# qinzheng93/GeoTransformer

Hardware: NVIDIA H100
Metric: point-cloud pairs/sec (3DMatch-shape synth) (higher is better)
Workload: dtype f32

## Files before the change

geotransformer_b200/_lib.py:

```python
import ctypes
import os
import threading

import torch

_HERE = os.path.dirname(os.path.abspath(__file__))
LIB_PATH = os.path.join(_HERE, 'libgeob200.so')
_lib = None

c_void_p, c_int64, c_int32, c_float, c_double, c_size_t, c_int = (
    ctypes.c_void_p, ctypes.c_int64, ctypes.c_int32, ctypes.c_float, ctypes.c_double, ctypes.c_size_t, ctypes.c_int)

SIGNATURES = {}


def _sig(name, restype, *argtypes):
    SIGNATURES[name] = (restype, list(argtypes))


P, I64, I32, F, D, SZ = c_void_p, c_int64, c_int32, c_float, c_double, c_size_t
_sig('geob200_last_error', ctypes.c_char_p)
_sig('geob200_launch_count', ctypes.c_uint64)
_sig('geob200_grid_subsample_workspace_bytes', SZ, I64, I64)
_sig('geob200_grid_subsample', c_int, P, I64, P, I64, F, P, P, P, SZ, P)
# ... 91 lines not shown
_sig('geob200_feature_corr_indices', c_int, P, P, P, P, I64, I64, I32, P, P, P, P, P)
_sig('geob200_ransac_features_batched_workspace_bytes', SZ, I64, I64, I64, I64, I64)
_sig('geob200_ransac_features_batched', c_int, P, P, P, P, I64, I64, I64, I64, P, P, F, I64, I64, I64, ctypes.c_uint64, I64, P, P, P, P, P,
     P, P, P, P, P, P, P, P, P, SZ, P)
_sig('geob200_correspondence_metrics_batched_workspace_bytes', SZ, I64, I64)
_sig('geob200_correspondence_metrics_batched', c_int, P, P, I64, I64, P, P, I64, F, P, I64, P, SZ, P)
_sig('geob200_corr_order_batched', c_int, P, I64, I64, P, I64, P, P)
_sig('geob200_corr_select_batched', c_int, P, P, P, I64, I64, P, P, I64, I64, P, P, P, P, P)
_sig('geob200_sparse_correspondence_eval_batched_workspace_bytes', SZ, I64, I64, I64)
_sig('geob200_sparse_correspondence_eval_batched', c_int, P, P, I64, P, P, I64, P, I64, I64, I64, P, P, SZ, P)
_sig('geob200_registration_error_batched', c_int, P, I64, P, I64, P, P, I64, c_int, D, D, P, P)
_sig('geob200_weighted_procrustes_counts', c_int, P, P, P, I64, I64, P, F, F, P, P)

_sig('geob200_linear_profile_enable', c_int, c_int)
_sig('geob200_set_split_k', c_int, c_int)
_sig('geob200_set_linear_persistent', c_int, c_int)
_sig('geob200_linear_profile_read', I64, I64, P, P)
_sig('geob200_backbone_workspace_bytes', SZ, P, P)
_sig('geob200_backbone_forward_batched', c_int, P, P, P, P, P, P, P, P, P, P, P, P, SZ, P, SZ, P, I64, P, P)
_sig('geob200_cloud_max_count', c_int, P, I64, I64, I64, I64, P, P, P)
_sig('geob200_transformer_batched_workspace_bytes', SZ, I64, P, I64, I64, I64)
_sig('geob200_transformer_forward_batched', c_int, P, I64, I64, I64, P, I64, P, P, P, P, SZ, P)
_sig('geob200_attention_batched_workspace_bytes', SZ, P, I64, I64)
_sig('geob200_attention_batched', c_int, P, I64, I64, I64, I64, I64, I64, I64, P, SZ, P)
_sig('geob200_attention_batched_keeps_probs', c_int, P, I64, I64, I64)
_sig('geob200_superpoint_targets_batched_workspace_bytes', SZ, I64)
_sig('geob200_superpoint_targets_batched', c_int, P, P, P, I64, P, F, I64, ctypes.c_uint64, ctypes.c_uint64, I64, P, P, P, P, SZ, P)
_sig('geob200_nonfinite_check', c_int, P, P, I64, I64, P, P)
_sig('geob200_batch_loss_weights', c_int, P, I64, I64, P, P, P, P, P)
_sig('geob200_kpconv_group_norm_batched', c_int, P, P, P, P, I64, I64, I64, P, I64, P, P, I64, I64, F, I64, P, P, F, c_int, F, P, P, P,
# ... 82 lines not shown
```

geotransformer_b200/csrc/common.cuh:

```cuda
#pragma once
#include <cuda_runtime.h>
#include <stdint.h>
#include <stdio.h>

namespace geob200 {

void set_error(const char* fmt, ...);
void count_launches(int n);
int ensure_max_smem(const void* kernel);

#define GEOB_CHECK_CUDA(expr)                                                                   \
    do {                                                                                        \
        cudaError_t _e = (expr);                                                                \
        if (_e != cudaSuccess) {                                                                \
            geob200::set_error("%s:%d CUDA error %s: %s", __FILE__, __LINE__, #expr,            \
                               cudaGetErrorString(_e));                                         \
            return -1;                                                                          \
        }                                                                                       \
    } while (0)

#define GEOB_CHECK_LAUNCH()                                                                     \
    do {                                                                                        \
        cudaError_t _e = cudaGetLastError();                                                    \
        if (_e != cudaSuccess) {                                                                \
// ... 39 lines not shown
    return v[0];
}

struct GnFuse {
    int groups;
    int slot_width;
    double* partial;
};

constexpr int GEOB_MAX_CLOUDS = 64;
struct GnSeg {
    int n_clouds;
    int n_pairs;
    int start[GEOB_MAX_CLOUDS + 1];
};
size_t fused_group_norm_workspace_bytes_batched(int64_t n_rows, int64_t channels, int64_t groups, int64_t n_pairs);
int group_norm_impl(const float* x, int64_t n_rows, int64_t channels, int64_t groups, const float* gamma, const float* beta, float eps,
                    const float* residual, int leaky, float slope, float* y, void* workspace, size_t workspace_bytes, void* stream,
                    const GnSeg* seg);
int linear_group_norm_impl(const float* x, int64_t ldx, const float* weight, const float* bias, int64_t m, int64_t n, int64_t k,
                           int64_t groups, const float* gamma, const float* beta, float eps, const float* residual, int leaky,
                           float slope, float* pre_norm, float* y, void* workspace, size_t workspace_bytes, void* stream,
                           const GnSeg* seg, const float* w_img = nullptr);
int kpconv_group_norm_impl(const float* s_feats, const float* q_points, const float* s_points, const int64_t* neighbors,
                           int64_t n_query, int64_t n_support, int64_t n_neighbors, const float* kernel_points, int64_t n_kernel,
                           const float* weights_t, const float* bias, int64_t c_in, int64_t c_out, float sigma, int64_t groups,
                           const float* gamma, const float* beta, float eps, int leaky, float slope, float* pre_norm, float* y,
                           void* gn_workspace, size_t gn_workspace_bytes, void* workspace, size_t workspace_bytes, void* stream,
                           const GnSeg* seg, const float* w_img = nullptr);
int linear_img(const float* x, int64_t ldx, const float* weight, const float* w_img, const float* bias, float* y, int64_t ldy,
               int64_t m, int64_t n, int64_t k, int relu, void* stream);
int kpconv_tc_impl(const float* s_feats, const float* q_points, const float* s_points, const int64_t* neighbors, int64_t n_query,
                   int64_t n_support, int64_t n_neighbors, const float* kernel_points, int64_t n_kernel, const float* weights_t,
                   const float* w_img, const float* bias, int64_t c_in, int64_t c_out, float sigma, float* out, void* workspace,
                   size_t workspace_bytes, void* stream);

int maxpool_seg(const float* x, const int64_t* neighbors, int64_t n_query, int64_t n_support, int64_t n_neighbors, int64_t channels,
                float* y, const GnSeg* seg, const int* cloud_max, void* stream);

struct Segs {
    int n;
    int max;
    int start[GEOB_MAX_CLOUDS];
    int count[GEOB_MAX_CLOUDS];
};
int segs_from_counts(Segs* s, int64_t n, const int64_t* counts);
// ... 54 lines not shown
```

geotransformer_b200/csrc/kpconv.cu:

```cuda
#include "common.cuh"
#include "geob200.h"
#include "kpconv.cuh"

namespace geob200 {

constexpr int TQ = 32;
constexpr int CC = 32;

__global__ void __launch_bounds__(256) kpconv_c1_kernel(const float* __restrict__ feats, const float* __restrict__ q_pts,
                                                        const float* __restrict__ s_pts, const long long* __restrict__ nbr,
                                                        int H, const float* __restrict__ kp, const float* __restrict__ W,
                                                        const float* __restrict__ bias, float sigma, int Ns, int M, int Cout,
                                                        float* __restrict__ out) {
    __shared__ float kp_s[KP * 3];
    __shared__ float wk_s[16][KP_PAD];
    __shared__ float np_s[16];
    if (threadIdx.x < KP * 3) kp_s[threadIdx.x] = kp[threadIdx.x];
    __syncthreads();
    const int lane = threadIdx.x & 31, warp = threadIdx.x >> 5;
    const int sub = lane >> 4, sl = lane & 15;
    const int slot = warp * 2 + sub;
    const int m = blockIdx.x * 16 + slot;
    const bool live = m < M;
    float acc[KP];
// ... 781 lines not shown
    const int lane = threadIdx.x & 31;
    const int m = blockIdx.x * 8 + (threadIdx.x >> 5);
    if (m >= M) return;
    const long long idx = up[(long long)m * up_stride];
    float* yr = y + (long long)m * (C1 + C2);
    for (int c = lane; c < C1; c += 32) yr[c] = (idx < Ns) ? x[idx * C1 + c] : 0.f;
    if (skip != nullptr)
        for (int c = lane; c < C2; c += 32) yr[C1 + c] = skip[(long long)m * C2 + c];
}

}

using namespace geob200;

namespace geob200 {
int linear_tc(const float* x, int64_t ldx, const float* w, int64_t ldw, const float* w_img, const float* bias, const float* row_scale, float* y, int64_t ldy,
              int64_t m, int64_t n, int64_t k, int relu, cudaStream_t st, const GnFuse* gn = nullptr);
static int g_linear_mode = 1;
}

extern "C" {

void geob200_set_linear_mode(int mode) { g_linear_mode = mode; }

size_t geob200_kpconv_workspace_bytes(int64_t n_support) { return (size_t)n_support + 256; }

size_t geob200_kpconv_tc_workspace_bytes(int64_t n_query, int64_t n_support, int64_t c_in) {
    return align_up((size_t)n_support, 256) + align_up((size_t)n_query * 4, 256) + (size_t)n_query * KP * (size_t)c_in * 4 + 1024;
}

int geob200_kpconv_tc(const float* s_feats, const float* q_points, const float* s_points, const int64_t* neighbors, int64_t n_query,
                      int64_t n_support, int64_t n_neighbors, const float* kernel_points, int64_t n_kernel, const float* weights_t,
// ... 18 lines not shown
    Arena ar(workspace, workspace_bytes);
    unsigned char* pos = ar.take<unsigned char>(n_support);
    float* inv_count = ar.take<float>(n_query);
    float* wf = ar.take<float>((size_t)n_query * KP * c_in);
    row_positive_kernel<<<(unsigned)((n_support + 7) / 8), 256, 0, st>>>(s_feats, (int)n_support, (int)c_in, pos);
    launch_kpconv_gather(s_feats, pos, q_points, s_points, (const long long*)neighbors, (int)n_neighbors, kernel_points, sigma,
                         (int)n_support, (int)n_query, (int)c_in, wf, inv_count, st);
    GEOB_CHECK_LAUNCH();
    count_launches(2);
    const int rc = linear_tc(wf, KP * c_in, weights_t, KP * c_in, w_img, bias, inv_count, out, c_out, n_query, c_out, KP * c_in, 0, st);
    GEOB_REQUIRE(rc == 0, "kpconv_tc: tensor-core GEMM rejected the shape");
    return 0;
}

int linear_img(const float* x, int64_t ldx, const float* weight, const float* w_img, const float* bias, float* y, int64_t ldy,
               int64_t m, int64_t n, int64_t k, int relu, void* stream) {
    if (g_linear_mode == 1 && m > 0 && n > 0 && k > 0) {
        const int rc = linear_tc(x, ldx, weight, k, w_img, bias, nullptr, y, ldy, m, n, k, relu, (cudaStream_t)stream);
        if (rc <= 0) return rc;
    }
    return geob200_linear(x, ldx, weight, bias, y, ldy, m, n, k, relu, stream);
}
}

extern "C" {

int geob200_kpconv(const float* s_feats, const float* q_points, const float* s_points, const int64_t* neighbors,
                   int64_t n_query, int64_t n_support, int64_t n_neighbors, const float* kernel_points, int64_t n_kernel,
                   const float* weights, const float* bias, int64_t c_in, int64_t c_out, float sigma, float* out,
                   void* workspace, size_t workspace_bytes, void* stream) {
    cudaStream_t st = (cudaStream_t)stream;
// ... 193 lines not shown
    return 0;
}

int geob200_linear_group_norm(const float* x, int64_t ldx, const float* weight, const float* bias, int64_t m, int64_t n, int64_t k,
                              int64_t groups, const float* gamma, const float* beta, float eps, const float* residual, int leaky,
                              float slope, float* pre_norm, float* y, void* workspace, size_t workspace_bytes, void* stream) {
    return geob200::linear_group_norm_impl(x, ldx, weight, bias, m, n, k, groups, gamma, beta, eps, residual, leaky, slope, pre_norm, y,
                                           workspace, workspace_bytes, stream, nullptr);
}
}

namespace geob200 {
int linear_group_norm_impl(const float* x, int64_t ldx, const float* weight, const float* bias, int64_t m, int64_t n, int64_t k,
                           int64_t groups, const float* gamma, const float* beta, float eps, const float* residual, int leaky,
                           float slope, float* pre_norm, float* y, void* workspace, size_t workspace_bytes, void* stream,
                           const GnSeg* seg, const float* w_img) {
    cudaStream_t st = (cudaStream_t)stream;
    const int64_t np = (seg != nullptr && seg->n_pairs > 1) ? seg->n_pairs : 1;
    GEOB_REQUIRE(m > 0 && n > 0 && k > 0 && groups > 0 && n % groups == 0 && n % 4 == 0, "linear_group_norm: bad shape");
    GEOB_REQUIRE(workspace_bytes >= (np > 1 ? fused_group_norm_workspace_bytes_batched(m, n, groups, np)
                                            : geob200_fused_group_norm_workspace_bytes(m, n, groups)), "linear_group_norm: workspace too small");
    if (g_linear_mode == 1) {
        const GnWs w = gn_carve(workspace, workspace_bytes, groups, np);
        GnFuse gn{(int)groups, 0, w.partial};
        const int rc = linear_tc(x, ldx, weight, k, w_img, bias, nullptr, pre_norm, n, m, n, k, 0, st, &gn);
        if (rc < 0) return rc;
        if (rc == 0) {
            if (np > 1) {
                launch_gn_seg_apply(pre_norm, w, gamma, beta, residual, y, m, n, groups, eps, leaky, slope, *seg, st);
            } else {
                launch_gn_apply(pre_norm, w, gamma, beta, residual, y, m, n, groups, eps, leaky, slope, st);
                count_launches(2);
            }
            GEOB_CHECK_LAUNCH();
            return 0;
        }
    }
    int rc = linear_img(x, ldx, weight, w_img, bias, pre_norm, n, m, n, k, 0, stream);
    if (rc != 0) return rc;
    return group_norm_impl(pre_norm, m, n, groups, gamma, beta, eps, residual, leaky, slope, y, workspace, workspace_bytes, stream, seg);
}
// ... 152 lines not shown
```

geotransformer_b200/csrc/linear_tc.cu:

```cuda
#include <cuda.h>

#include <cstdlib>
#include <mutex>
#include <vector>

#include "common.cuh"
#include "geob200.h"
#include "hopper.cuh"

namespace geob200 {
namespace ltc {

using namespace hop;

constexpr int BM = 128;
constexpr int KC = 32;
constexpr int TILE_A = BM * 128;
constexpr int TILE_B = 128 * 128;
constexpr int STAGE = TILE_A + 2 * TILE_B;
constexpr int NSTAGE = 4;
constexpr int PRODUCER_WARP = 8;
constexpr int NTHREADS = (PRODUCER_WARP + 4) * 32;
constexpr int SMEM = NSTAGE * STAGE + 1024 + 256 + 8 * 128 * 8 + 512;

__global__ void __launch_bounds__(256) split_tf32_kernel(const float* __restrict__ w, long long ld, long long n, long long k,
                                                         float* __restrict__ out) {
    const long long nk = n * k;
    for (long long i = (long long)blockIdx.x * blockDim.x + threadIdx.x; i < nk; i += (long long)gridDim.x * blockDim.x) {
        const long long r = i / k, c = i % k;
        const float x = w[r * ld + c];
        const float hi = tf32_rn(x);
        out[i] = hi;
        out[nk + i] = x - hi;
    }
}

template <int BNI>
__global__ void __launch_bounds__(NTHREADS, 1) linear_tc_kernel(const __grid_constant__ CUtensorMap map_x,
                                                                const __grid_constant__ CUtensorMap map_w,
                                                                const float* __restrict__ bias, const float* __restrict__ row_scale,
                                                                float* __restrict__ Y, int ldy, int M, int N, int K, int BN, int relu,
                                                                GnFuse gn, float* __restrict__ splitk_out, int chunks_per_split,
                                                                int col_tiles, int row_tiles, int num_tiles) {
    constexpr int R = BNI / 2;
    extern __shared__ unsigned char smem_raw[];
    unsigned char* smem = (unsigned char*)(((uintptr_t)smem_raw + 1023) & ~(uintptr_t)1023);
    uint64_t* bars = (uint64_t*)(smem + NSTAGE * STAGE);
    uint64_t* full = bars;
    uint64_t* empty = bars + NSTAGE;
    float2* gn_sm = (float2*)(smem + NSTAGE * STAGE + 256);
    float* bias_s = (float*)(gn_sm + 8 * 128);
    const int warp = threadIdx.x >> 5, lane = threadIdx.x & 31;
    const int nk = (K + KC - 1) / KC;
    const int tiles_per_split = col_tiles * row_tiles;

    if (threadIdx.x == 0) {
        for (int s = 0; s < NSTAGE; ++s) { mbar_init(&full[s], 1); mbar_init(&empty[s], 8); }
        asm volatile("fence.mbarrier_init.release.cluster;" ::: "memory");
// ... 29 lines not shown
    const int wg = warp >> 2, wq = warp & 3;
    int s = 0;
    uint32_t ph = 0;
    for (int t = blockIdx.x; t < num_tiles; t += gridDim.x) {
        const int z = t / tiles_per_split, rem = t % tiles_per_split;
        const int ty = rem / col_tiles;
        const int m0 = ty * BM, n0 = (rem % col_tiles) * BN;
        const int kc0 = z * chunks_per_split, kc1 = min(nk, kc0 + chunks_per_split);
        asm volatile("bar.sync 1, 256;" ::: "memory");
        if (threadIdx.x < 128) bias_s[threadIdx.x] = (bias != nullptr && (int)threadIdx.x < BN) ? __ldg(bias + n0 + threadIdx.x) : 0.f;
        asm volatile("bar.sync 1, 256;" ::: "memory");

        float acc[R], cor[R];
#pragma unroll
        for (int i = 0; i < R; ++i) { acc[i] = 0.f; cor[i] = 0.f; }
        const int g = lane >> 2, tq = lane & 3;
        const int a_off = (wg * 64 + wq * 16 + g) * 128 + tq * 4;
        for (int kc = kc0; kc < kc1; ++kc) {
            mbar_wait(&full[s], ph);
            unsigned char* st = smem + s * STAGE;
            uint32_t f[2][KC / 8][4];
#pragma unroll
            for (int kk = 0; kk < KC / 8; ++kk)
#pragma unroll
                for (int e = 0; e < 4; ++e) {
                    const int j = 2 * kk + (e >> 1);
                    const float x = *reinterpret_cast<const float*>(st + a_off + (e & 1) * 8 * 128 + ((j ^ g) << 4));
                    const float hi = tf32_rn(x);
                    f[0][kk][e] = __float_as_uint(hi);
                    f[1][kk][e] = __float_as_uint(x - hi);
                }
            const uint32_t sb = smem_u32(st + TILE_A);
            const uint64_t b_hi = make_desc(sb), b_lo = make_desc(sb + TILE_B);
            wgmma_fence();
#pragma unroll
            for (int kk = 0; kk < KC / 8; ++kk) {
                const uint64_t adv = (uint64_t)(kk * 2);
                const uint32_t accum = (kc == kc0 && kk == 0) ? 0u : 1u;
                wgmma_tf32_rs<BNI>(acc, f[0][kk], b_hi + adv, accum);
                wgmma_tf32_rs<BNI>(cor, f[0][kk], b_lo + adv, accum);
                wgmma_tf32_rs<BNI>(cor, f[1][kk], b_hi + adv, 1u);
            }
            wgmma_commit();
            wgmma_wait<0>();
            __syncwarp();
            if (lane == 0) mbar_arrive(&empty[s]);
            if (++s == NSTAGE) { s = 0; ph ^= 1u; }
        }
        reg_fence(acc);
        reg_fence(cor);

        const int r0 = m0 + wg * 64 + wq * 16 + (lane >> 2);
        const int c0 = 2 * (lane & 3);
        float rs[2];
#pragma unroll
        for (int h = 0; h < 2; ++h) rs[h] = (row_scale != nullptr && r0 + 8 * h < M) ? row_scale[r0 + 8 * h] : 1.0f;
        if (splitk_out != nullptr) {
#pragma unroll
            for (int j = 0; j < BNI / 8; ++j)
#pragma unroll
                for (int h = 0; h < 2; ++h) {
                    const int m = r0 + 8 * h, col = 8 * j + c0;
                    if (m < M && col < BN)
                        *reinterpret_cast<float2*>(splitk_out + ((long long)z * M + m) * N + n0 + col) =
                            make_float2(acc[4 * j + 2 * h] + cor[4 * j + 2 * h], acc[4 * j + 2 * h + 1] + cor[4 * j + 2 * h + 1]);
                }
            continue;
        }
// ... 105 lines not shown
    cuuint32_t box[2] = {(cuuint32_t)KC, (cuuint32_t)box_rows};
    cuuint32_t estr[2] = {1, 1};
    CUresult r = fn(map, CU_TENSOR_MAP_DATA_TYPE_FLOAT32, 2, (void*)base, gdim, gstride, box, estr, CU_TENSOR_MAP_INTERLEAVE_NONE,
                    CU_TENSOR_MAP_SWIZZLE_128B, CU_TENSOR_MAP_L2_PROMOTION_L2_128B, CU_TENSOR_MAP_FLOAT_OOB_FILL_NONE);
    if (r != CUDA_SUCCESS) { set_error("cuTensorMapEncodeTiled failed with CUresult %d", (int)r); return -1; }
    return 0;
}

}

struct ProfRec { cudaEvent_t a, b; long long m, n, k; };
static std::vector<ProfRec> g_prof;
static std::mutex g_prof_mu;
static bool g_prof_on = false;
static bool g_splitk_on = true;
static bool g_persistent_on = true;

struct StreamWs { void* ptr; size_t bytes; };
static std::vector<std::pair<cudaStream_t, StreamWs>> g_split_ws, g_wimg_ws;
static std::mutex g_split_mu;
static float* stream_scratch(std::vector<std::pair<cudaStream_t, StreamWs>>& pool, cudaStream_t st, size_t bytes) {
    std::lock_guard<std::mutex> lk(g_split_mu);
    for (auto& e : pool)
        if (e.first == st) {
            if (e.second.bytes >= bytes) return (float*)e.second.ptr;
            cudaFreeAsync(e.second.ptr, st);
            e.second = {nullptr, 0};
            if (cudaMallocAsync(&e.second.ptr, bytes * 2, st) != cudaSuccess) return nullptr;
            e.second.bytes = bytes * 2;
            return (float*)e.second.ptr;
// ... 2 lines not shown
    const size_t cap = bytes * 2 > (16u << 20) ? bytes * 2 : (16u << 20);
    if (cudaMallocAsync(&w.ptr, cap, st) != cudaSuccess) return nullptr;
    w.bytes = cap;
    pool.push_back({st, w});
    return (float*)w.ptr;
}

static void launch_split_tf32(const float* w, int64_t ld, int64_t n, int64_t k, float* out, cudaStream_t st) {
    const long long nk = (long long)n * k;
    long long blocks = (nk + 255) / 256;
    if (blocks > 4LL * num_sms()) blocks = 4LL * num_sms();
    ltc::split_tf32_kernel<<<(unsigned)(blocks > 0 ? blocks : 1), 256, 0, st>>>(w, ld, n, k, out);
    count_launches(1);
}

int linear_tc(const float* x, int64_t ldx, const float* w, int64_t ldw, const float* w_img, const float* bias, const float* row_scale,
              float* y, int64_t ldy, int64_t m, int64_t n, int64_t k, int relu, cudaStream_t st, const GnFuse* gn) {
    if (m < 64 || n < 32 || (n % 16) != 0 || (k % 4) != 0 || (ldx % 4) != 0) return 1;
    if ((reinterpret_cast<uintptr_t>(x) & 15) || (reinterpret_cast<uintptr_t>(w_img) & 15)) return 1;
    if (w_img == nullptr && ((ldw % 4) != 0 || (reinterpret_cast<uintptr_t>(w) & 15))) return 1;
    if (n > 128 && (n % 128) != 0) return 1;
    const int BN = (int)(n >= 128 ? 128 : n);
    const int col_tiles = (int)(n / BN), row_tiles = (int)((m + ltc::BM - 1) / ltc::BM);
    GnFuse g{};
    if (gn != nullptr) {
        g = *gn;
        const int64_t cpg = n / g.groups;
        if (g.groups <= 0 || n % g.groups != 0 || (cpg < 32 ? (32 % cpg) != 0 : (cpg % 32) != 0 || (BN % cpg) != 0) || relu) return 1;
        g.slot_width = (int)(cpg < 32 ? cpg : 32);
    }
    const int nk = (int)((k + ltc::KC - 1) / ltc::KC);
    const int tiles = col_tiles * row_tiles;
    int splits = 1;
    if (g_splitk_on && tiles * 2 <= num_sms() && nk >= 16) {
        splits = nk / 8;
        if (splits > num_sms() / tiles) splits = num_sms() / tiles;
        if (splits > 16) splits = 16;
        if (splits < 2) splits = 1;
    }
    if (gn != nullptr && splits > 1) return 1;
    int cps = nk;
    float* part = nullptr;
    if (splits > 1) {
        cps = (nk + splits - 1) / splits;
        splits = (nk + cps - 1) / cps;
        part = stream_scratch(g_split_ws, st, (size_t)splits * (size_t)m * (size_t)n * sizeof(float));
        if (part == nullptr) { splits = 1; cps = nk; }
    }
    float* img = nullptr;
    if (w_img == nullptr) {
        img = stream_scratch(g_wimg_ws, st, (size_t)2 * (size_t)n * (size_t)k * sizeof(float));
        if (img == nullptr) { set_error("linear_tc: weight image scratch allocation failed"); return -1; }
        w_img = img;
    }
    CUtensorMap mx, mw;
    if (ltc::encode_map(&mx, x, m, k, ldx, ltc::BM)) return -1;
    if (ltc::encode_map(&mw, w_img, 2 * n, k, k, BN)) return -1;
    ProfRec rec{};
    const bool prof = g_prof_on;
    if (prof) {
        cudaEventCreate(&rec.a);
        cudaEventCreate(&rec.b);
        rec.m = m; rec.n = n; rec.k = k;
        cudaEventRecord(rec.a, st);
    }
    if (img != nullptr) launch_split_tf32(w, ldw, n, k, img, st);
    const int num_tiles = tiles * splits;
    const bool persistent = g_persistent_on && splits == 1 && tiles > num_sms();
    const unsigned grid = (unsigned)(persistent ? num_sms() : num_tiles);
    const void* kern = BN <= 32 ? (const void*)ltc::linear_tc_kernel<32> : BN <= 64 ? (const void*)ltc::linear_tc_kernel<64>
                                                                                      : (const void*)ltc::linear_tc_kernel<128>;
    if (ensure_max_smem(kern)) return -1;
#define GEOB_LTC_LAUNCH(BNI)                                                                                                  \
    ltc::linear_tc_kernel<BNI><<<grid, ltc::NTHREADS, ltc::SMEM, st>>>(mx, mw, bias, row_scale, y, (int)ldy, (int)m, (int)n, (int)k, \
                                                                       BN, relu, g, part, cps, col_tiles, row_tiles, num_tiles)
    if (BN <= 32) GEOB_LTC_LAUNCH(32);
    else if (BN <= 64) GEOB_LTC_LAUNCH(64);
    else GEOB_LTC_LAUNCH(128);
#undef GEOB_LTC_LAUNCH
    if (part != nullptr) {
        const long long mn = (long long)m * n;
        ltc::splitk_reduce_kernel<<<(unsigned)((mn / 4 + 255) / 256), 256, 0, st>>>(part, splits, mn, (int)n, bias, row_scale, y, (int)ldy, relu);
        count_launches(1);
    }
    if (prof) {
        cudaEventRecord(rec.b, st);
        std::lock_guard<std::mutex> lk(g_prof_mu);
        g_prof.push_back(rec);
    }
    GEOB_CHECK_LAUNCH();
    count_launches(1);
    return 0;
}

}

extern "C" {

int geob200_set_linear_persistent(int on) {
    geob200::g_persistent_on = on != 0;
    return 0;
}

int geob200_split_tf32(const float* w, int64_t ld, int64_t n, int64_t k, float* out, void* stream) {
    GEOB_REQUIRE(n > 0 && k > 0 && ld >= k, "split_tf32: bad shape (%lld x %lld, ld %lld)", (long long)n, (long long)k, (long long)ld);
    geob200::launch_split_tf32(w, ld, n, k, out, (cudaStream_t)stream);
    GEOB_CHECK_LAUNCH();
    return 0;
}

int geob200_set_split_k(int on) {
    geob200::g_splitk_on = on != 0;
    return 0;
}

int geob200_linear_profile_enable(int on) {
    std::lock_guard<std::mutex> lk(geob200::g_prof_mu);
    for (auto& r : geob200::g_prof) { cudaEventDestroy(r.a); cudaEventDestroy(r.b); }
    geob200::g_prof.clear();
    geob200::g_prof_on = on != 0;
    return 0;
}

int64_t geob200_linear_profile_read(int64_t capacity, int64_t* shapes, float* ms) {
    std::lock_guard<std::mutex> lk(geob200::g_prof_mu);
    int64_t n = 0;
    for (auto& r : geob200::g_prof) {
        if (n >= capacity) break;
        if (cudaEventSynchronize(r.b) != cudaSuccess) break;
// ... 11 lines not shown
```

geotransformer_b200/csrc/native.cu:

```cuda
#include "common.cuh"
#include "geob200.h"

namespace geob200 {

struct Ctx {
    Arena ar;
    void* gn_ws;
    size_t gn_ws_bytes;
    void* stream;
    int groups;
    Ctx(void* p, size_t n) : ar(p, n) {}
    float* fl(int64_t rows, int64_t ch) { return ar.take<float>((size_t)rows * (size_t)ch); }
};

#define TRY(expr)                  \
    do {                           \
        int _rc = (expr);          \
        if (_rc != 0) return _rc;  \
    } while (0)

static int run_kpconv(Ctx& c, const geob200_kpconv_t& k, const float* s_feats, const float* q_pts, const float* s_pts,
                      const int64_t* nbr, int64_t m, int64_t ns, int64_t h, float* out) {
    const bool tc = (k.c_in % 32 == 0) && (k.c_out % 16 == 0) && k.c_out >= 32 && (k.c_out <= 128 || k.c_out % 128 == 0) && m >= 64 &&
                    k.weights_t != nullptr;
// ... 27 lines not shown
        const size_t wb = geob200_kpconv_tc_workspace_bytes(m, ns, k.c_in);
        const size_t mark = c.ar.off;
        void* ws = c.ar.take<char>(wb);
        GEOB_REQUIRE(c.ar.ok(), "native: arena too small (kpconv)");
        TRY(kpconv_group_norm_impl(s_feats, q_pts, s_pts, nbr, m, ns, h, k.kernel_points, 15, k.weights_t, k.bias, k.c_in, k.c_out,
                                   k.sigma, c.groups, n.gamma, n.beta, 1e-5f, 1, 0.1f, y, out, c.gn_ws, c.gn_ws_bytes, ws, wb, c.stream, seg,
                                   k.weights_img));
        c.ar.off = mark;
        return 0;
    }
    TRY(run_kpconv(c, k, s_feats, q_pts, s_pts, nbr, m, ns, h, y));
    return group_norm_impl(y, m, k.c_out, c.groups, n.gamma, n.beta, 1e-5f, nullptr, 1, 0.1f, out, c.gn_ws, c.gn_ws_bytes, c.stream, seg);
}

static int run_unary(Ctx& c, const geob200_linear_t& l, const geob200_norm_t& n, const float* x, int64_t rows, const float* residual,
                     int leaky, float* out, const GnSeg* seg) {
    float* t = c.fl(rows, l.c_out);
    GEOB_REQUIRE(c.ar.ok(), "native: arena too small (unary)");
    TRY(linear_group_norm_impl(x, l.c_in, l.weight, l.bias, rows, l.c_out, l.c_in, c.groups, n.gamma, n.beta, 1e-5f, residual, leaky,
                               0.1f, t, out, c.gn_ws, c.gn_ws_bytes, c.stream, seg, l.weight_img));
    return 0;
}

static int run_resblock(Ctx& c, const geob200_resblock_t& b, const float* feats, int64_t ns, const float* q_pts, const float* s_pts,
                        const int64_t* nbr, int64_t m, int64_t h, float* out, const GnSeg* seg_s, const GnSeg* seg_q,
                        const int* cloud_max = nullptr) {
    const float* x = feats;
    if (b.has_unary1) {
        float* u = c.fl(ns, b.unary1.c_out);
        TRY(run_unary(c, b.unary1, b.norm1, feats, ns, nullptr, 1, u, seg_s));
        x = u;
    }
    float* yn = c.fl(m, b.conv.c_out);
    GEOB_REQUIRE(c.ar.ok(), "native: arena too small (resblock)");
    TRY(run_kpconv_norm(c, b.conv, b.norm_conv, x, q_pts, s_pts, nbr, m, ns, h, yn, seg_q));
    const float* sc = feats;
// ... 78 lines not shown
                         sg[lvl - 1], sg[lvl], sub_cloud_max != nullptr ? sub_cloud_max[lvl - 1] : nullptr));
        const geob200_resblock_t& b2 = net->blocks[bi++];
        float* o2 = c.fl(m, b2.unary2.c_out);
        TRY(run_resblock(c, b2, o1, m, points[lvl], points[lvl], neighbors[lvl], m, neighbor_width[lvl], o2, sg[lvl], sg[lvl]));
        const geob200_resblock_t& b3 = net->blocks[bi++];
        float* o3 = (lvl == S - 1) ? out_feats[0] : c.fl(m, b3.unary2.c_out);
        TRY(run_resblock(c, b3, o2, m, points[lvl], points[lvl], neighbors[lvl], m, neighbor_width[lvl], o3, sg[lvl], sg[lvl]));
        enc[lvl] = o3; enc_ch[lvl] = b3.unary2.c_out;
    }
    const float* latent = enc[S - 1];
    int64_t latent_ch = enc_ch[S - 1];
    int oi = 1;
    for (int lvl = S - 1; lvl >= net->finest_decoder; --lvl) {
        const int64_t m = level_rows[lvl - 1], ns = level_rows[lvl];
        const int64_t c2 = enc_ch[lvl - 1];
        float* cat = c.fl(m, latent_ch + c2);
        GEOB_REQUIRE(c.ar.ok(), "native: arena too small (decoder)");
        TRY(geob200_upsample_concat(latent, upsampling[lvl - 1], upsampling_width[lvl - 1], ns, enc[lvl - 1], m, latent_ch, c2, cat, stream));
        const geob200_linear_t& l = net->decoders[S - 1 - lvl];
        float* o = out_feats[oi++];
        if (lvl == net->finest_decoder) {
            TRY(linear_img(cat, l.c_in, l.weight, l.weight_img, l.bias, o, l.c_out, m, l.c_out, l.c_in, 0, stream));
        } else {
            TRY(run_unary(c, l, net->decoder_norms[S - 1 - lvl], cat, m, nullptr, 1, o, sg[lvl - 1]));
        }
        latent = o; latent_ch = l.c_out;
    }
    GEOB_REQUIRE(c.ar.ok(), "native: arena too small");
    return 0;
}


static int run_tail(Ctx& c, const geob200_tlayer_t& L, const float* hidden, const float* inp, int64_t rows, int64_t ch, float* out) {
    float* h = c.fl(rows, ch);
    float* x = c.fl(rows, ch);
    float* y1 = c.fl(rows, 2 * ch);
    float* y2 = c.fl(rows, ch);
    GEOB_REQUIRE(c.ar.ok(), "native: arena too small (transformer tail)");
    TRY(linear_img(hidden, ch, L.att_linear.weight, L.att_linear.weight_img, L.att_linear.bias, h, ch, rows, ch, ch, 0, c.stream));
    TRY(geob200_add_layernorm(h, inp, L.att_norm.gamma, L.att_norm.beta, rows, ch, 1e-5f, x, c.stream));
// ... 95 lines not shown
```

include/geob200.h:

```cpp
#ifndef GEOB200_H
#define GEOB200_H

#include <stddef.h>
#include <stdint.h>

#ifdef __cplusplus
extern "C" {
#endif

const char* geob200_last_error(void);
uint64_t geob200_launch_count(void);


size_t geob200_grid_subsample_workspace_bytes(int64_t n_points, int64_t batch);
int geob200_grid_subsample(const float* points, int64_t n_points, const int64_t* lengths_h, int64_t batch, float voxel,
                           float* s_points, int64_t* s_lengths, void* workspace, size_t workspace_bytes, void* stream);

size_t geob200_radius_search_workspace_bytes(int64_t n_query, int64_t n_support, int64_t batch);
int geob200_radius_search(const float* q_points, int64_t n_query, const float* s_points, int64_t n_support,
                          const int64_t* q_lengths_h, const int64_t* s_lengths_h, int64_t batch, float radius,
                          int64_t width, int64_t* out, int32_t* counts, int32_t* max_count, void* workspace,
                          size_t workspace_bytes, void* stream);

int geob200_neighbor_histogram(const int64_t* neighbors, int64_t n_rows, int64_t width, int64_t n_support, int64_t hist_n,
// ... 294 lines not shown
                                float* ref_out, float* src_out, float* scores_out, int32_t* count_out, void* stream);
size_t geob200_sparse_correspondence_eval_batched_workspace_bytes(int64_t n_pairs, int64_t m_cap, int64_t n_cap);
int geob200_sparse_correspondence_eval_batched(const int64_t* ref_node_corr_indices, const int64_t* src_node_corr_indices, int64_t pred_cap,
                                               const int32_t* pred_count, const int64_t* gt_node_corr_indices, int64_t gt_cap,
                                               const int32_t* gt_count, int64_t n_pairs, int64_t m_cap, int64_t n_cap, double* out,
                                               void* workspace, size_t workspace_bytes, void* stream);
int geob200_registration_error_batched(const float* gt_transforms, int64_t gt_ld, const float* est_transforms, int64_t est_ld,
                                       const float* covariances, const int32_t* has_covariance, int64_t n_pairs, int mode,
                                       double threshold0, double threshold1, double* out, void* stream);
int geob200_weighted_procrustes_counts(const float* src_points, const float* ref_points, const float* weights, int64_t batch,
                                       int64_t capacity, const int32_t* counts, float weight_thresh, float eps, float* transforms,
                                       void* stream);

int geob200_linear_profile_enable(int on);
int geob200_set_split_k(int on);
int geob200_set_linear_persistent(int on);
int64_t geob200_linear_profile_read(int64_t capacity, int64_t* shapes, float* ms);

#define GEOB200_MAX_STAGES 6
typedef struct { const float* weight; const float* bias; int64_t c_in, c_out; const float* weight_img; } geob200_linear_t;
typedef struct { const float* gamma; const float* beta; } geob200_norm_t;
typedef struct { const float* weights; const float* weights_t; const float* bias; const float* kernel_points;
                 int64_t c_in, c_out; float sigma; const float* weights_img; } geob200_kpconv_t;
typedef struct {
    int32_t has_unary1, has_shortcut, strided, reserved;
    int64_t c_in;
    geob200_linear_t unary1; geob200_norm_t norm1;
    geob200_kpconv_t conv;   geob200_norm_t norm_conv;
    geob200_linear_t unary2; geob200_norm_t norm2;
    geob200_linear_t shortcut; geob200_norm_t norm_sc;
// ... 69 lines not shown
```

Measured before the change: 432.4.

## Fuse decoder upsample-concat into linear via coarse-level partial GEMM carry

Instead of materialising the upsampled-and-concatenated decoder input, the decoder linear is split. The latent part of the weight is multiplied once at the coarse level (ns+1 rows) and the hi/lo accumulators are stored in a carry buffer. The fine-level GEMM then seeds its accumulators by gathering the carry rows through the upsampling indices and only multiplies the skip-connection columns. This removes the concat kernel and the redundant latent-channel FLOPs on the fine rows, at the cost of an extra launch, a gathered float4 load per row, and a fallback path when the shape constraints are not met.

```diff
diff --git a/geotransformer_b200/_lib.py b/geotransformer_b200/_lib.py
--- a/geotransformer_b200/_lib.py
+++ b/geotransformer_b200/_lib.py
@@ -129,6 +129,7 @@
 
 _sig('geob200_linear_profile_enable', c_int, c_int)
 _sig('geob200_set_split_k', c_int, c_int)
+_sig('geob200_decoder_carry_count', ctypes.c_uint64)
 _sig('geob200_set_linear_persistent', c_int, c_int)
 _sig('geob200_linear_profile_read', I64, I64, P, P)
 _sig('geob200_backbone_workspace_bytes', SZ, P, P)
diff --git a/geotransformer_b200/csrc/common.cuh b/geotransformer_b200/csrc/common.cuh
--- a/geotransformer_b200/csrc/common.cuh
+++ b/geotransformer_b200/csrc/common.cuh
@@ -77,6 +77,16 @@
     int n_pairs;
     int start[GEOB_MAX_CLOUDS + 1];
 };
+struct DecoderCarry {
+    const float* latent;
+    int64_t ns, latent_ch;
+    const int64_t* up;
+    int64_t up_stride;
+    float* carry;
+};
+int linear_tc(const float* x, int64_t ldx, const float* w, int64_t ldw, const float* w_img, const float* bias, const float* row_scale,
+              float* y, int64_t ldy, int64_t m, int64_t n, int64_t k, int relu, cudaStream_t st, const GnFuse* gn = nullptr,
+              const DecoderCarry* dc = nullptr);
 size_t fused_group_norm_workspace_bytes_batched(int64_t n_rows, int64_t channels, int64_t groups, int64_t n_pairs);
 int group_norm_impl(const float* x, int64_t n_rows, int64_t channels, int64_t groups, const float* gamma, const float* beta, float eps,
                     const float* residual, int leaky, float slope, float* y, void* workspace, size_t workspace_bytes, void* stream,
@@ -84,7 +94,7 @@
 int linear_group_norm_impl(const float* x, int64_t ldx, const float* weight, const float* bias, int64_t m, int64_t n, int64_t k,
                            int64_t groups, const float* gamma, const float* beta, float eps, const float* residual, int leaky,
                            float slope, float* pre_norm, float* y, void* workspace, size_t workspace_bytes, void* stream,
-                           const GnSeg* seg, const float* w_img = nullptr);
+                           const GnSeg* seg, const float* w_img = nullptr, const DecoderCarry* dc = nullptr);
 int kpconv_group_norm_impl(const float* s_feats, const float* q_points, const float* s_points, const int64_t* neighbors,
                            int64_t n_query, int64_t n_support, int64_t n_neighbors, const float* kernel_points, int64_t n_kernel,
                            const float* weights_t, const float* bias, int64_t c_in, int64_t c_out, float sigma, int64_t groups,
@@ -92,7 +102,7 @@
                            void* gn_workspace, size_t gn_workspace_bytes, void* workspace, size_t workspace_bytes, void* stream,
                            const GnSeg* seg, const float* w_img = nullptr);
 int linear_img(const float* x, int64_t ldx, const float* weight, const float* w_img, const float* bias, float* y, int64_t ldy,
-               int64_t m, int64_t n, int64_t k, int relu, void* stream);
+               int64_t m, int64_t n, int64_t k, int relu, void* stream, const DecoderCarry* dc = nullptr);
 int kpconv_tc_impl(const float* s_feats, const float* q_points, const float* s_points, const int64_t* neighbors, int64_t n_query,
                    int64_t n_support, int64_t n_neighbors, const float* kernel_points, int64_t n_kernel, const float* weights_t,
                    const float* w_img, const float* bias, int64_t c_in, int64_t c_out, float sigma, float* out, void* workspace,
diff --git a/geotransformer_b200/csrc/kpconv.cu b/geotransformer_b200/csrc/kpconv.cu
--- a/geotransformer_b200/csrc/kpconv.cu
+++ b/geotransformer_b200/csrc/kpconv.cu
@@ -819,8 +819,6 @@
 using namespace geob200;
 
 namespace geob200 {
-int linear_tc(const float* x, int64_t ldx, const float* w, int64_t ldw, const float* w_img, const float* bias, const float* row_scale, float* y, int64_t ldy,
-              int64_t m, int64_t n, int64_t k, int relu, cudaStream_t st, const GnFuse* gn = nullptr);
 static int g_linear_mode = 1;
 }
 
@@ -869,7 +867,10 @@
 }
 
 int linear_img(const float* x, int64_t ldx, const float* weight, const float* w_img, const float* bias, float* y, int64_t ldy,
-               int64_t m, int64_t n, int64_t k, int relu, void* stream) {
+               int64_t m, int64_t n, int64_t k, int relu, void* stream, const DecoderCarry* dc) {
+    if (dc != nullptr)
+        return g_linear_mode == 1 ? linear_tc(x, ldx, weight, k, w_img, bias, nullptr, y, ldy, m, n, k, relu, (cudaStream_t)stream, nullptr, dc)
+                                  : 1;
     if (g_linear_mode == 1 && m > 0 && n > 0 && k > 0) {
         const int rc = linear_tc(x, ldx, weight, k, w_img, bias, nullptr, y, ldy, m, n, k, relu, (cudaStream_t)stream);
         if (rc <= 0) return rc;
@@ -1093,17 +1094,18 @@
 int linear_group_norm_impl(const float* x, int64_t ldx, const float* weight, const float* bias, int64_t m, int64_t n, int64_t k,
                            int64_t groups, const float* gamma, const float* beta, float eps, const float* residual, int leaky,
                            float slope, float* pre_norm, float* y, void* workspace, size_t workspace_bytes, void* stream,
-                           const GnSeg* seg, const float* w_img) {
+                           const GnSeg* seg, const float* w_img, const DecoderCarry* dc) {
     cudaStream_t st = (cudaStream_t)stream;
     const int64_t np = (seg != nullptr && seg->n_pairs > 1) ? seg->n_pairs : 1;
     GEOB_REQUIRE(m > 0 && n > 0 && k > 0 && groups > 0 && n % groups == 0 && n % 4 == 0, "linear_group_norm: bad shape");
     GEOB_REQUIRE(workspace_bytes >= (np > 1 ? fused_group_norm_workspace_bytes_batched(m, n, groups, np)
                                             : geob200_fused_group_norm_workspace_bytes(m, n, groups)), "linear_group_norm: workspace too small");
+    if (dc != nullptr && g_linear_mode != 1) return 1;
     if (g_linear_mode == 1) {
         const GnWs w = gn_carve(workspace, workspace_bytes, groups, np);
         GnFuse gn{(int)groups, 0, w.partial};
-        const int rc = linear_tc(x, ldx, weight, k, w_img, bias, nullptr, pre_norm, n, m, n, k, 0, st, &gn);
-        if (rc < 0) return rc;
+        const int rc = linear_tc(x, ldx, weight, k, w_img, bias, nullptr, pre_norm, n, m, n, k, 0, st, &gn, dc);
+        if (rc < 0 || (rc == 1 && dc != nullptr)) return rc;
         if (rc == 0) {
             if (np > 1) {
                 launch_gn_seg_apply(pre_norm, w, gamma, beta, residual, y, m, n, groups, eps, leaky, slope, *seg, st);
diff --git a/geotransformer_b200/csrc/linear_tc.cu b/geotransformer_b200/csrc/linear_tc.cu
--- a/geotransformer_b200/csrc/linear_tc.cu
+++ b/geotransformer_b200/csrc/linear_tc.cu
@@ -1,5 +1,6 @@
 #include <cuda.h>
 
+#include <atomic>
 #include <cstdlib>
 #include <mutex>
 #include <vector>
@@ -35,13 +36,22 @@
     }
 }
 
+enum { CARRY_NONE = 0, CARRY_OUT = 1, CARRY_IN = 2 };
+struct Carry {
+    int mode;
+    int ns;
+    float* buf;
+    const long long* up;
+    long long up_stride;
+};
+
 template <int BNI>
 __global__ void __launch_bounds__(NTHREADS, 1) linear_tc_kernel(const __grid_constant__ CUtensorMap map_x,
                                                                 const __grid_constant__ CUtensorMap map_w,
                                                                 const float* __restrict__ bias, const float* __restrict__ row_scale,
                                                                 float* __restrict__ Y, int ldy, int M, int N, int K, int BN, int relu,
                                                                 GnFuse gn, float* __restrict__ splitk_out, int chunks_per_split,
-                                                                int col_tiles, int row_tiles, int num_tiles) {
+                                                                int col_tiles, int row_tiles, int num_tiles, Carry carry) {
     constexpr int R = BNI / 2;
     extern __shared__ unsigned char smem_raw[];
     unsigned char* smem = (unsigned char*)(((uintptr_t)smem_raw + 1023) & ~(uintptr_t)1023);
@@ -101,6 +111,27 @@
         float acc[R], cor[R];
 #pragma unroll
         for (int i = 0; i < R; ++i) { acc[i] = 0.f; cor[i] = 0.f; }
+        const int r0 = m0 + wg * 64 + wq * 16 + (lane >> 2);
+        const int c0 = 2 * (lane & 3);
+        if (carry.mode == CARRY_IN) {
+            long long src[2] = {0, 0};
+#pragma unroll
+            for (int h = 0; h < 2; ++h)
+                if (r0 + 8 * h < M) src[h] = carry.up[(long long)(r0 + 8 * h) * carry.up_stride];
+#pragma unroll
+            for (int h = 0; h < 2; ++h) {
+                if (r0 + 8 * h >= M) continue;
+                const long long row = (unsigned long long)src[h] >= (unsigned long long)carry.ns ? carry.ns : src[h];
+                const float* rp = carry.buf + row * 2 * N + 2 * (n0 + c0);
+#pragma unroll
+                for (int j = 0; j < BNI / 8; ++j)
+                    if (8 * j + c0 < BN) {
+                        const float4 v = *reinterpret_cast<const float4*>(rp + 16 * j);
+                        acc[4 * j + 2 * h] = v.x; acc[4 * j + 2 * h + 1] = v.y;
+                        cor[4 * j + 2 * h] = v.z; cor[4 * j + 2 * h + 1] = v.w;
+                    }
+            }
+        }
         const int g = lane >> 2, tq = lane & 3;
         const int a_off = (wg * 64 + wq * 16 + g) * 128 + tq * 4;
         for (int kc = kc0; kc < kc1; ++kc) {
@@ -123,7 +154,7 @@
 #pragma unroll
             for (int kk = 0; kk < KC / 8; ++kk) {
                 const uint64_t adv = (uint64_t)(kk * 2);
-                const uint32_t accum = (kc == kc0 && kk == 0) ? 0u : 1u;
+                const uint32_t accum = (kc == kc0 && kk == 0 && carry.mode != CARRY_IN) ? 0u : 1u;
                 wgmma_tf32_rs<BNI>(acc, f[0][kk], b_hi + adv, accum);
                 wgmma_tf32_rs<BNI>(cor, f[0][kk], b_lo + adv, accum);
                 wgmma_tf32_rs<BNI>(cor, f[1][kk], b_hi + adv, 1u);
@@ -137,8 +168,19 @@
         reg_fence(acc);
         reg_fence(cor);
 
-        const int r0 = m0 + wg * 64 + wq * 16 + (lane >> 2);
-        const int c0 = 2 * (lane & 3);
+        if (carry.mode == CARRY_OUT) {
+#pragma unroll
+            for (int j = 0; j < BNI / 8; ++j)
+#pragma unroll
+                for (int h = 0; h < 2; ++h) {
+                    const int m = r0 + 8 * h, col = 8 * j + c0;
+                    if (m < M && col < BN) {
+                        *reinterpret_cast<float4*>(carry.buf + (long long)m * 2 * N + 2 * (n0 + col)) =
+                            make_float4(acc[4 * j + 2 * h], acc[4 * j + 2 * h + 1], cor[4 * j + 2 * h], cor[4 * j + 2 * h + 1]);
+                    }
+                }
+            continue;
+        }
         float rs[2];
 #pragma unroll
         for (int h = 0; h < 2; ++h) rs[h] = (row_scale != nullptr && r0 + 8 * h < M) ? row_scale[r0 + 8 * h] : 1.0f;
@@ -274,6 +316,7 @@
 static std::mutex g_prof_mu;
 static bool g_prof_on = false;
 static bool g_splitk_on = true;
+static std::atomic<unsigned long long> g_decoder_carry{0};
 static bool g_persistent_on = true;
 
 struct StreamWs { void* ptr; size_t bytes; };
@@ -306,8 +349,37 @@
     count_launches(1);
 }
 
+static void prof_begin(ProfRec* rec, int64_t m, int64_t n, int64_t k, cudaStream_t st) {
+    cudaEventCreate(&rec->a);
+    cudaEventCreate(&rec->b);
+    rec->m = m; rec->n = n; rec->k = k;
+    cudaEventRecord(rec->a, st);
+}
+static void prof_end(ProfRec* rec, cudaStream_t st) {
+    cudaEventRecord(rec->b, st);
+    std::lock_guard<std::mutex> lk(g_prof_mu);
+    g_prof.push_back(*rec);
+}
+
+static void launch_ltc(const CUtensorMap& mx, const CUtensorMap& mw, const float* bias, const float* row_scale, float* y, int64_t ldy,
+                       int64_t m, int64_t n, int64_t k, int BN, int relu, const GnFuse& g, float* part, int cps, int splits,
+                       const ltc::Carry& carry, cudaStream_t st) {
+    const int col_tiles = (int)(n / BN), row_tiles = (int)((m + ltc::BM - 1) / ltc::BM);
+    const int num_tiles = col_tiles * row_tiles * splits;
+    const bool persistent = g_persistent_on && splits == 1 && col_tiles * row_tiles > num_sms();
+    const unsigned grid = (unsigned)(persistent ? num_sms() : num_tiles);
+#define GEOB_LTC_LAUNCH(BNI)                                                                                                  \
+    ltc::linear_tc_kernel<BNI><<<grid, ltc::NTHREADS, ltc::SMEM, st>>>(mx, mw, bias, row_scale, y, (int)ldy, (int)m, (int)n, (int)k, \
+                                                                       BN, relu, g, part, cps, col_tiles, row_tiles, num_tiles, carry)
+    if (BN <= 32) GEOB_LTC_LAUNCH(32);
+    else if (BN <= 64) GEOB_LTC_LAUNCH(64);
+    else GEOB_LTC_LAUNCH(128);
+#undef GEOB_LTC_LAUNCH
+    count_launches(1);
+}
+
 int linear_tc(const float* x, int64_t ldx, const float* w, int64_t ldw, const float* w_img, const float* bias, const float* row_scale,
-              float* y, int64_t ldy, int64_t m, int64_t n, int64_t k, int relu, cudaStream_t st, const GnFuse* gn) {
+              float* y, int64_t ldy, int64_t m, int64_t n, int64_t k, int relu, cudaStream_t st, const GnFuse* gn, const DecoderCarry* dc) {
     if (m < 64 || n < 32 || (n % 16) != 0 || (k % 4) != 0 || (ldx % 4) != 0) return 1;
     if ((reinterpret_cast<uintptr_t>(x) & 15) || (reinterpret_cast<uintptr_t>(w_img) & 15)) return 1;
     if (w_img == nullptr && ((ldw % 4) != 0 || (reinterpret_cast<uintptr_t>(w) & 15))) return 1;
@@ -323,8 +395,13 @@
     }
     const int nk = (int)((k + ltc::KC - 1) / ltc::KC);
     const int tiles = col_tiles * row_tiles;
+    const bool splitk = g_splitk_on && tiles * 2 <= num_sms() && nk >= 16;
+    if (dc != nullptr) {
+        const int64_t lc = dc->latent_ch;
+        if (splitk || lc <= 0 || lc % ltc::KC != 0 || lc >= k || dc->ns < 1 || (reinterpret_cast<uintptr_t>(dc->latent) & 15)) return 1;
+    }
     int splits = 1;
-    if (g_splitk_on && tiles * 2 <= num_sms() && nk >= 16) {
+    if (splitk) {
         splits = nk / 8;
         if (splits > num_sms() / tiles) splits = num_sms() / tiles;
         if (splits > 16) splits = 16;
@@ -345,43 +422,48 @@
         if (img == nullptr) { set_error("linear_tc: weight image scratch allocation failed"); return -1; }
         w_img = img;
     }
+    const void* kern = BN <= 32 ? (const void*)ltc::linear_tc_kernel<32> : BN <= 64 ? (const void*)ltc::linear_tc_kernel<64>
+                                                                                      : (const void*)ltc::linear_tc_kernel<128>;
+    if (ensure_max_smem(kern)) return -1;
+    const bool prof = g_prof_on;
+    ltc::Carry carry{ltc::CARRY_NONE, 0, nullptr, nullptr, 0};
+    if (dc != nullptr) {
+        const int64_t lc = dc->latent_ch, ns = dc->ns;
+        CUtensorMap mxl, mwl, mx, mw;
+        if (ltc::encode_map(&mxl, dc->latent, ns, lc, lc, ltc::BM)) return -1;
+        if (ltc::encode_map(&mwl, w_img, 2 * n, lc, k, BN)) return -1;
+        if (ltc::encode_map(&mx, x, m, k - lc, ldx, ltc::BM)) return -1;
+        if (ltc::encode_map(&mw, w_img + lc, 2 * n, k - lc, k, BN)) return -1;
+        ProfRec rec{};
+        if (prof) prof_begin(&rec, ns + 1, n, lc, st);
+        if (img != nullptr) launch_split_tf32(w, ldw, n, k, img, st);
+        carry = ltc::Carry{ltc::CARRY_OUT, (int)ns, dc->carry, nullptr, 0};
+        launch_ltc(mxl, mwl, nullptr, nullptr, nullptr, 0, ns + 1, n, lc, BN, 0, GnFuse{}, nullptr, (int)((lc + ltc::KC - 1) / ltc::KC), 1,
+                   carry, st);
+        if (prof) { prof_end(&rec, st); prof_begin(&rec, m, n, k - lc, st); }
+        carry.mode = ltc::CARRY_IN;
+        carry.up = (const long long*)dc->up;
+        carry.up_stride = dc->up_stride;
+        launch_ltc(mx, mw, bias, row_scale, y, ldy, m, n, k - lc, BN, relu, g, nullptr, (int)((k - lc + ltc::KC - 1) / ltc::KC), 1, carry, st);
+        if (prof) prof_end(&rec, st);
+        GEOB_CHECK_LAUNCH();
+        g_decoder_carry.fetch_add(1);
+        return 0;
+    }
     CUtensorMap mx, mw;
     if (ltc::encode_map(&mx, x, m, k, ldx, ltc::BM)) return -1;
     if (ltc::encode_map(&mw, w_img, 2 * n, k, k, BN)) return -1;
     ProfRec rec{};
-    const bool prof = g_prof_on;
-    if (prof) {
-        cudaEventCreate(&rec.a);
-        cudaEventCreate(&rec.b);
-        rec.m = m; rec.n = n; rec.k = k;
-        cudaEventRecord(rec.a, st);
-    }
+    if (prof) prof_begin(&rec, m, n, k, st);
     if (img != nullptr) launch_split_tf32(w, ldw, n, k, img, st);
-    const int num_tiles = tiles * splits;
-    const bool persistent = g_persistent_on && splits == 1 && tiles > num_sms();
-    const unsigned grid = (unsigned)(persistent ? num_sms() : num_tiles);
-    const void* kern = BN <= 32 ? (const void*)ltc::linear_tc_kernel<32> : BN <= 64 ? (const void*)ltc::linear_tc_kernel<64>
-                                                                                      : (const void*)ltc::linear_tc_kernel<128>;
-    if (ensure_max_smem(kern)) return -1;
-#define GEOB_LTC_LAUNCH(BNI)                                                                                                  \
-    ltc::linear_tc_kernel<BNI><<<grid, ltc::NTHREADS, ltc::SMEM, st>>>(mx, mw, bias, row_scale, y, (int)ldy, (int)m, (int)n, (int)k, \
-                                                                       BN, relu, g, part, cps, col_tiles, row_tiles, num_tiles)
-    if (BN <= 32) GEOB_LTC_LAUNCH(32);
-    else if (BN <= 64) GEOB_LTC_LAUNCH(64);
-    else GEOB_LTC_LAUNCH(128);
-#undef GEOB_LTC_LAUNCH
+    launch_ltc(mx, mw, bias, row_scale, y, ldy, m, n, k, BN, relu, g, part, cps, splits, carry, st);
     if (part != nullptr) {
         const long long mn = (long long)m * n;
         ltc::splitk_reduce_kernel<<<(unsigned)((mn / 4 + 255) / 256), 256, 0, st>>>(part, splits, mn, (int)n, bias, row_scale, y, (int)ldy, relu);
         count_launches(1);
     }
-    if (prof) {
-        cudaEventRecord(rec.b, st);
-        std::lock_guard<std::mutex> lk(g_prof_mu);
-        g_prof.push_back(rec);
-    }
+    if (prof) prof_end(&rec, st);
     GEOB_CHECK_LAUNCH();
-    count_launches(1);
     return 0;
 }
 
@@ -405,6 +487,8 @@
     geob200::g_splitk_on = on != 0;
     return 0;
 }
+
+uint64_t geob200_decoder_carry_count(void) { return geob200::g_decoder_carry.load(); }
 
 int geob200_linear_profile_enable(int on) {
     std::lock_guard<std::mutex> lk(geob200::g_prof_mu);
diff --git a/geotransformer_b200/csrc/native.cu b/geotransformer_b200/csrc/native.cu
--- a/geotransformer_b200/csrc/native.cu
+++ b/geotransformer_b200/csrc/native.cu
@@ -65,12 +65,11 @@
 }
 
 static int run_unary(Ctx& c, const geob200_linear_t& l, const geob200_norm_t& n, const float* x, int64_t rows, const float* residual,
-                     int leaky, float* out, const GnSeg* seg) {
+                     int leaky, float* out, const GnSeg* seg, const DecoderCarry* dc = nullptr, int64_t ldx = 0) {
     float* t = c.fl(rows, l.c_out);
     GEOB_REQUIRE(c.ar.ok(), "native: arena too small (unary)");
-    TRY(linear_group_norm_impl(x, l.c_in, l.weight, l.bias, rows, l.c_out, l.c_in, c.groups, n.gamma, n.beta, 1e-5f, residual, leaky,
-                               0.1f, t, out, c.gn_ws, c.gn_ws_bytes, c.stream, seg, l.weight_img));
-    return 0;
+    return linear_group_norm_impl(x, dc != nullptr ? ldx : l.c_in, l.weight, l.bias, rows, l.c_out, l.c_in, c.groups, n.gamma, n.beta, 1e-5f,
+                                  residual, leaky, 0.1f, t, out, c.gn_ws, c.gn_ws_bytes, c.stream, seg, l.weight_img, dc);
 }
 
 static int run_resblock(Ctx& c, const geob200_resblock_t& b, const float* feats, int64_t ns, const float* q_pts, const float* s_pts,
@@ -179,16 +178,23 @@
     for (int lvl = S - 1; lvl >= net->finest_decoder; --lvl) {
         const int64_t m = level_rows[lvl - 1], ns = level_rows[lvl];
         const int64_t c2 = enc_ch[lvl - 1];
-        float* cat = c.fl(m, latent_ch + c2);
+        const geob200_linear_t& l = net->decoders[S - 1 - lvl];
+        const bool last = lvl == net->finest_decoder;
+        float* o = out_feats[oi++];
+        const size_t mark = c.ar.off;
+        const DecoderCarry dc{latent, ns, latent_ch, upsampling[lvl - 1], upsampling_width[lvl - 1], c.fl(2 * (ns + 1), l.c_out)};
         GEOB_REQUIRE(c.ar.ok(), "native: arena too small (decoder)");
-        TRY(geob200_upsample_concat(latent, upsampling[lvl - 1], upsampling_width[lvl - 1], ns, enc[lvl - 1], m, latent_ch, c2, cat, stream));
-        const geob200_linear_t& l = net->decoders[S - 1 - lvl];
-        float* o = out_feats[oi++];
-        if (lvl == net->finest_decoder) {
-            TRY(linear_img(cat, l.c_in, l.weight, l.weight_img, l.bias, o, l.c_out, m, l.c_out, l.c_in, 0, stream));
-        } else {
-            TRY(run_unary(c, l, net->decoder_norms[S - 1 - lvl], cat, m, nullptr, 1, o, sg[lvl - 1]));
+        int rc = last ? linear_img(enc[lvl - 1], c2, l.weight, l.weight_img, l.bias, o, l.c_out, m, l.c_out, l.c_in, 0, stream, &dc)
+                      : run_unary(c, l, net->decoder_norms[S - 1 - lvl], enc[lvl - 1], m, nullptr, 1, o, sg[lvl - 1], &dc, c2);
+        if (rc == 1) {
+            c.ar.off = mark;
+            float* cat = c.fl(m, latent_ch + c2);
+            GEOB_REQUIRE(c.ar.ok(), "native: arena too small (decoder)");
+            TRY(geob200_upsample_concat(latent, upsampling[lvl - 1], upsampling_width[lvl - 1], ns, enc[lvl - 1], m, latent_ch, c2, cat, stream));
+            rc = last ? linear_img(cat, l.c_in, l.weight, l.weight_img, l.bias, o, l.c_out, m, l.c_out, l.c_in, 0, stream)
+                      : run_unary(c, l, net->decoder_norms[S - 1 - lvl], cat, m, nullptr, 1, o, sg[lvl - 1]);
         }
+        TRY(rc);
         latent = o; latent_ch = l.c_out;
     }
     GEOB_REQUIRE(c.ar.ok(), "native: arena too small");
diff --git a/include/geob200.h b/include/geob200.h
--- a/include/geob200.h
+++ b/include/geob200.h
@@ -332,6 +332,7 @@
 
 int geob200_linear_profile_enable(int on);
 int geob200_set_split_k(int on);
+uint64_t geob200_decoder_carry_count(void);
 int geob200_set_linear_persistent(int on);
 int64_t geob200_linear_profile_read(int64_t capacity, int64_t* shapes, float* ms);
 
```

After: 446.3, median of 6. +3.2%, better.
